# NickTravers/NeuralNetworkLibrary

Measured on AMD Instinct MI355X. Metric: ResNet-34 224x224 training throughput (Learner.train1minibatch, fwd+loss+bwd+optimizer), higher is better.
Workload: dtype f32; 1 GPU; DogsCats ResNet-34 classifier, 224x224, bs=64 per GPU, SGD momentum 0.9, fp32; global_batch=64, image_size=224, parallelism=dp1

## Files before the change

### include/nnl.h

```cpp
#ifndef NNL_H_
#define NNL_H_

#include <stddef.h>
#include <stdint.h>

#ifdef __cplusplus
extern "C" {
#endif

typedef enum {
  NNL_OK = 0,
  NNL_ERR_INVALID_ARG = -1,
  NNL_ERR_HIP = -2,
  NNL_ERR_UNSUPPORTED = -3,
  NNL_ERR_WORKSPACE = -4
} nnl_status_t;

int nnl_version(void);
const char* nnl_last_error(void);
int nnl_reload_env(void);

enum { NNL_PROF_CONV_FWD = 0, NNL_PROF_CONV_DGRAD = 1, NNL_PROF_CONV_WGRAD = 2, NNL_PROF_EMBDOT = 3,
       NNL_PROF_TABULAR = 4, NNL_PROF_RETINA_LOSS = 5, NNL_PROF_LSTM = 6, NNL_PROF_SOFTMAX_CE = 7,
       NNL_PROF_ELEMENTWISE = 8, NNL_PROF_GEMM = 9, NNL_PROF_OPTIM = 10, NNL_PROF_KINDS = 11 };
// ... 62 lines not shown
                            int H, int W, int C, int K, int relu, int flip, void* stream);
int nnl_debug_conv_plan_times(int N, int H, int W, int C, int K, double* out);

int nnl_debug_route_record(int enable);
int nnl_debug_route_collect(char* out, size_t n);
size_t nnl_conv2d_wgrad_workspace_bytes(const nnl_conv_geom_t* g);
int nnl_conv2d_wgrad(const float* x, const float* dy, float* dw, const nnl_conv_geom_t* g, void* workspace,
                     size_t workspace_bytes, void* stream);
size_t nnl_colsum_workspace_bytes(int64_t rows, int64_t cols);
int nnl_sum_tensors(const float* const* src, int n, float* out, int64_t numel, void* stream);
int nnl_colsum(const float* a, float* out, int64_t rows, int64_t cols, void* workspace, size_t workspace_bytes,
               void* stream);
int nnl_relu_gate_colsum(const float* dy, const float* y, float* g, float* colsum, int64_t rows, int64_t cols, void* workspace,
                         size_t workspace_bytes, void* stream);
int nnl_act_gate_colsum(const float* dy, const float* y, float* g, float* colsum, int64_t rows, int64_t cols, int act,
                        void* workspace, size_t workspace_bytes, void* stream);

size_t nnl_bn_workspace_bytes(int64_t rows, int64_t C);
int nnl_bn_fwd(const float* x, const float* gamma, const float* beta, const float* residual, float* y,
               float* save_mean, float* save_invstd, float* running_mean, float* running_var, int64_t rows,
               int64_t C, float eps, float momentum, int training, int relu, int64_t* num_batches_tracked,
               uint32_t* relu_mask, const float* ext_partials, int64_t ext_rows, const float* ext_pivot, float* pivot_out,
               void* workspace, size_t workspace_bytes, void* stream);
int nnl_bn_bwd(const float* dy, const float* y, const uint32_t* relu_mask, const float* x, const float* gamma,
               const float* mean, const float* invstd, float* dx, float* dres, float* dgamma, float* dbeta, int64_t rows,
               int64_t C, int training, int relu, void* workspace, size_t workspace_bytes, void* stream);

int nnl_bn_relu_maxpool_supported(int64_t C);
int nnl_bn_relu_maxpool_fwd(const float* x, const float* gamma, const float* beta, float* y, uint8_t* idx, float* save_mean,
                            float* save_invstd, float* save_scale, float* save_shift, float* running_mean, float* running_var,
                            int64_t N, int64_t H, int64_t W, int64_t C, int64_t P, int64_t Q, int ks, int stride, int pad, float eps,
                            float momentum, int training, int64_t* num_batches_tracked, void* workspace, size_t workspace_bytes,
                            void* stream);
int nnl_bn_relu_maxpool_bwd(const float* dpool, const float* y, const uint8_t* idx, const float* x, const float* gamma,
                            const float* beta, const float* mean, const float* invstd, const float* scale, const float* shift,
                            float* dx, float* dgamma, float* dbeta,
                            int64_t N, int64_t H, int64_t W, int64_t C, int64_t P, int64_t Q, int ks, int stride, int pad,
                            int training, void* workspace, size_t workspace_bytes, void* stream);

int nnl_debug_bn_plan(int64_t rows, int64_t C, int64_t N, int64_t H, int64_t W, int64_t P, int64_t Q, int32_t* out10);

int nnl_bn_sync_stats(const float* x, float* stats, int64_t rows, int64_t C, void* workspace, size_t workspace_bytes,
                      void* stream);
int nnl_bn_sync_fwd(const float* x, const float* all_stats, int world, const float* gamma, const float* beta,
                    const float* residual, float* y, float* save_mean, float* save_invstd, float* running_mean,
                    float* running_var, int64_t rows, int64_t C, float eps, float momentum, int relu,
                    int64_t* num_batches_tracked, uint32_t* relu_mask, void* workspace, size_t workspace_bytes, void* stream);
int nnl_bn_sync_bwd_reduce(const float* dy, const float* y, const uint32_t* relu_mask, const float* x, const float* mean,
                           const float* invstd, float* sums, int64_t rows, int64_t C, int relu, void* workspace,
                           size_t workspace_bytes, void* stream);
int nnl_bn_sync_bwd(const float* dy, const float* y, const uint32_t* relu_mask, const float* x, const float* gamma,
                    const float* mean, const float* invstd, const float* local_sums, const float* global_sums,
                    const float* all_stats,
                    int world, float* dx, float* dres, float* dgamma, float* dbeta, int64_t rows, int64_t C, int relu,
                    void* workspace, size_t workspace_bytes, void* stream);

int nnl_maxpool2d_fwd(const float* x, float* y, uint8_t* idx, int64_t N, int64_t H, int64_t W, int64_t C, int64_t P,
                      int64_t Q, int ksize, int stride, int pad, void* stream);
int nnl_maxpool2d_bwd(const float* dy, const uint8_t* idx, float* dx, int64_t N, int64_t H, int64_t W, int64_t C,
                      int64_t P, int64_t Q, int ksize, int stride, int pad, void* stream);
int nnl_concat_pool_fwd(const float* x, float* out, int32_t* argmax, int64_t N, int64_t HW, int64_t C, void* stream);
int nnl_concat_pool_bwd(const float* dout, const int32_t* argmax, float* dx, int64_t N, int64_t HW, int64_t C, void* stream);

int nnl_bbox_decode(const float* anchors, const float* reg, const float* clas, int64_t bs, int64_t A, int64_t K,
                    const float* mean4, const float* std4, float thresh, float width, float height, float* cand_boxes,
                    int32_t* cand_classes, float* cand_scores, int32_t* cand_order, int32_t* cand_count, void* stream);
// ... 165 lines not shown
```

### neuralnetworklibrary_amd/_lib.py

```python
import ctypes as C
import os

import torch

_HERE = os.path.dirname(os.path.abspath(__file__))
LIB_PATH = os.environ.get('NNL_LIB_PATH') or os.path.join(_HERE, 'libnnl_hip.so')

if not os.path.exists(LIB_PATH):
    raise ImportError(
        f"{LIB_PATH} not found: build it with `python -c 'import __graft_entry__ as g; g.build()'` "
        "(or `make -C neuralnetworklibrary_amd/csrc`). There is no CPU fallback for the HIP hot path.")

lib = C.CDLL(LIB_PATH)

c_p = C.c_void_p
i32, i64, f32, f64 = C.c_int32, C.c_int64, C.c_float, C.c_double
sz = C.c_size_t


class ConvGeom(C.Structure):
    _fields_ = [('N', i32), ('H', i32), ('W', i32), ('C', i32), ('K', i32), ('R', i32), ('S', i32),
                ('stride', i32), ('pad', i32), ('P', i32), ('Q', i32)]


# ... 15 lines not shown
                                     f32, f32, c_p, sz, c_p]),
    'nnl_conv2d_fwd_workspace_bytes': (sz, [C.POINTER(ConvGeom)]),
    'nnl_conv2d_dgrad_workspace_bytes': (sz, [C.POINTER(ConvGeom)]),
    'nnl_conv2d_tile_counters': (i64, []),
    'nnl_conv2d_wino_preferred': (C.c_int, [C.POINTER(ConvGeom), C.c_int]),
    'nnl_wino_filter_multi': (C.c_int, [c_p, c_p, i64, c_p]),
    'nnl_conv2d_fwd_pre': (C.c_int, [c_p, c_p, c_p, c_p, C.POINTER(ConvGeom), C.c_int, c_p, sz, c_p, c_p, c_p, C.POINTER(i32), c_p, c_p]),
    'nnl_conv2d_dgrad_pre': (C.c_int, [c_p, c_p, c_p, C.POINTER(ConvGeom), c_p, c_p, sz, c_p, c_p, c_p]),
    'nnl_debug_conv_wino_workspace_bytes': (sz, [C.c_int] * 5),
    'nnl_debug_conv_wino_fwd': (C.c_int, [c_p] * 6 + [sz, c_p, C.c_long, c_p, c_p] + [C.c_int] * 7 + [c_p]),
    'nnl_debug_conv_wino2_workspace_bytes': (sz, [C.c_int] * 5),
    'nnl_debug_conv_wino2_fwd': (C.c_int, [c_p] * 6 + [sz, c_p, C.c_long, c_p, c_p] + [C.c_int] * 7 + [c_p]),
    'nnl_debug_conv_plan_times': (C.c_int, [C.c_int] * 5 + [C.POINTER(C.c_double)]),
    'nnl_debug_route_record': (C.c_int, [C.c_int]),
    'nnl_debug_route_collect': (C.c_int, [C.c_char_p, sz]),
    'nnl_conv2d_fwd': (C.c_int, [c_p, c_p, c_p, c_p, C.POINTER(ConvGeom), C.c_int, c_p, sz, c_p, c_p, c_p, C.POINTER(i32), c_p]),
    'nnl_conv2d_weight_transpose': (C.c_int, [c_p, c_p, C.c_int, C.c_int, C.c_int, C.c_int, c_p]),
    'nnl_conv2d_weight_transpose_multi': (C.c_int, [c_p, c_p, i64, f64, c_p]),
    'nnl_conv2d_dgrad': (C.c_int, [c_p, c_p, c_p, C.POINTER(ConvGeom), c_p, c_p, sz, c_p, c_p]),
    'nnl_conv2d_wgrad_workspace_bytes': (sz, [C.POINTER(ConvGeom)]),
    'nnl_conv2d_wgrad': (C.c_int, [c_p, c_p, c_p, C.POINTER(ConvGeom), c_p, sz, c_p]),
    'nnl_colsum_workspace_bytes': (sz, [i64, i64]),
    'nnl_colsum': (C.c_int, [c_p, c_p, i64, i64, c_p, sz, c_p]),
    'nnl_relu_gate_colsum': (C.c_int, [c_p, c_p, c_p, c_p, i64, i64, c_p, sz, c_p]),
    'nnl_conv2d_fwd_add_up2': (C.c_int, [c_p, c_p, c_p, c_p, c_p, C.POINTER(ConvGeom), c_p]),
    'nnl_upsample2_bwd': (C.c_int, [c_p, c_p, i64, i64, i64, i64, c_p]),
    'nnl_act_gate_colsum': (C.c_int, [c_p, c_p, c_p, c_p, i64, i64, C.c_int, c_p, sz, c_p]),
    'nnl_maxpool2d_fwd': (C.c_int, [c_p, c_p, c_p, i64, i64, i64, i64, i64, i64, C.c_int, C.c_int, C.c_int, c_p]),
    'nnl_maxpool2d_bwd': (C.c_int, [c_p, c_p, c_p, i64, i64, i64, i64, i64, i64, C.c_int, C.c_int, C.c_int, c_p]),
    'nnl_sum_tensors': (C.c_int, [c_p, C.c_int, c_p, i64, c_p]),
    'nnl_bn_relu_maxpool_supported': (C.c_int, [i64]),
    'nnl_bn_relu_maxpool_fwd': (C.c_int, [c_p, c_p, c_p, c_p, c_p, c_p, c_p, c_p, c_p, c_p, c_p, i64, i64, i64, i64, i64, i64,
                                          C.c_int, C.c_int, C.c_int, f32, f32, C.c_int, c_p, c_p, sz, c_p]),
    'nnl_bn_relu_maxpool_bwd': (C.c_int, [c_p, c_p, c_p, c_p, c_p, c_p, c_p, c_p, c_p, c_p, c_p, c_p, c_p, i64, i64, i64, i64, i64, i64,
                                          C.c_int, C.c_int, C.c_int, C.c_int, c_p, sz, c_p]),
    'nnl_concat_pool_fwd': (C.c_int, [c_p, c_p, c_p, i64, i64, i64, c_p]),
    'nnl_concat_pool_bwd': (C.c_int, [c_p, c_p, c_p, i64, i64, i64, c_p]),
    'nnl_bbox_decode': (C.c_int, [c_p, c_p, c_p, i64, i64, i64, c_p, c_p, f32, f32, f32, c_p, c_p, c_p, c_p, c_p, c_p]),
    'nnl_bbox_decode_window': (C.c_int, [c_p, c_p, c_p, i64, i64, i64, c_p, c_p, f32, f32, f32, f32, f32, c_p, c_p, c_p, c_p, c_p, c_p]),
    'nnl_nms_workspace_bytes': (sz, [i64, i64]),
    'nnl_nms': (C.c_int, [c_p, c_p, c_p, c_p, c_p, i64, i64, i64, f32, c_p, c_p, c_p, c_p, c_p, sz, c_p]),
    'nnl_tta_bbox_merge': (C.c_int, [c_p, c_p, c_p, c_p, c_p, i64, i64, i64, c_p, c_p, c_p, c_p, c_p, c_p, c_p]),
    'nnl_tab_renorm': (C.c_int, [c_p, c_p, c_p, c_p, c_p, c_p, c_p, i64, i32, i32, f32, c_p, c_p]),
    'nnl_tab_gather_fwd': (C.c_int, [c_p, c_p, c_p, c_p, c_p, c_p, c_p, c_p, c_p, c_p, i64, i32, i32, i32, i32, c_p]),
    'nnl_tab_scatter_bwd_workspace_bytes': (sz, [i64, i32]),
    'nnl_tab_scatter_bwd': (C.c_int, [c_p, c_p, c_p, c_p, c_p, c_p, c_p, c_p, c_p, c_p, i64, c_p, i64, i32, i32, i32, i32, c_p, sz, c_p]),
    'nnl_tab_scan_bwd': (C.c_int, [c_p] * 12 + [i32, i32, i64, i32, i32, i32, i32, c_p]),
    'nnl_pad_cols': (C.c_int, [c_p, c_p, i64, i64, i64, c_p]),
    'nnl_keep_masks': (C.c_int, [c_p, c_p, i64, f32, c_p, i64, f32, c_p]),
    'nnl_linear_small_supported': (C.c_int, [i64]),
    'nnl_linear_small_fwd': (C.c_int, [c_p, c_p, c_p, c_p, i64, i64, i64, i64, c_p]),
    'nnl_linear_small_bwd_workspace_bytes': (sz, [i64, i64, i64]),
    'nnl_linear_small_bwd': (C.c_int, [c_p, c_p, c_p, c_p, c_p, c_p, i64, i64, i64, i64, c_p, sz, c_p]),
    'nnl_retina_loss_workspace_bytes': (sz, [i64, i64]),
    'nnl_retina_loss_fwd': (C.c_int, [c_p, c_p, c_p, c_p, c_p, c_p, c_p, c_p, i64, i64, i64, i64, f32, f32, f32, c_p, sz, c_p]),
    'nnl_retina_loss_bwd': (C.c_int, [c_p, c_p, c_p, c_p, c_p, c_p, c_p, c_p, c_p, c_p, i64, i64, i64, i64, f32, f32, f32, c_p]),
    'nnl_lstm_padded_hidden': (i64, [i64]),
    'nnl_lstm_padded_gates': (i64, [i64]),
    'nnl_lstm_workspace_bytes': (sz, [i64, i64, i64]),
    'nnl_lstm_fwd': (C.c_int, [c_p, c_p, c_p, c_p, c_p, c_p, c_p, i64, i64, i64, c_p, sz, c_p, c_p]),
    'nnl_lstm_bwd': (C.c_int, [c_p, c_p, c_p, c_p, c_p, c_p, c_p, c_p, c_p, c_p, i64, i64, i64, c_p, sz, c_p, c_p]),
    'nnl_debug_lstm_bptt2_plan': (C.c_int, [i64, i64, c_p]),
    'nnl_debug_lstm_plan': (C.c_int, [i64, i64, C.POINTER(i32)]),
    'nnl_embedding_rowmask_fwd': (C.c_int, [c_p, c_p, c_p, c_p, i64, i64, i64, c_p, c_p]),
    'nnl_embedding_rowmask_bwd_workspace_bytes': (sz, [i64]),
    'nnl_embedding_rowmask_bwd': (C.c_int, [c_p, c_p, c_p, c_p, i64, i64, i64, i64, c_p, sz, c_p]),
# ... 103 lines not shown
```

### neuralnetworklibrary_amd/csrc/batchnorm.hip

```cpp
#include "nnl_common.h"

namespace {

typedef float f32x4 __attribute__((ext_vector_type(4)));

template <int VEC> struct VecT;
template <> struct VecT<4> { typedef f32x4 type; };
template <> struct VecT<1> { typedef float type; };

template <int VEC> __device__ __forceinline__ float vget(const typename VecT<VEC>::type& v, int i);
template <> __device__ __forceinline__ float vget<4>(const f32x4& v, int i) { return v[i]; }
template <> __device__ __forceinline__ float vget<1>(const float& v, int i) { return v; }
template <int VEC> __device__ __forceinline__ void vset(typename VecT<VEC>::type& v, int i, float x);
template <> __device__ __forceinline__ void vset<4>(f32x4& v, int i, float x) { v[i] = x; }
template <> __device__ __forceinline__ void vset<1>(float& v, int i, float x) { v = x; }

constexpr int kBlock = 256;
constexpr int kMaxRowBlocks = 1024;
constexpr float kCentreAbove = 16.f;
constexpr int kFinLanes = 64;

struct Shape {
  int L;
  int rpb;
// ... 776 lines not shown
    long r = i / g.C4;
    const int w = (int)(r % g.W); r /= g.W;
    const int h = (int)(r % g.H);
    const int n = (int)(r / g.H);
    const f32x4 xv = reinterpret_cast<const f32x4*>(x)[i];
    const f32x4 gg = bnpool_grad(dpool, idx, xv, sc, sh, n, h, w, c4, g);
    f32x4 out;
#pragma unroll
    for (int e = 0; e < 4; ++e) out[e] = ca[e] * gg[e] + cb[e] * xv[e] + cc[e];
    reinterpret_cast<f32x4*>(dx)[i] = out;
  }
}

bool bnpool_ok(long C) { return C % 4 == 0 && C >= 4 && C <= 1024 && (kBlock % (C / 4)) == 0; }
unsigned bnpool_grid(long total) {
  long g = nnl_cdiv(total, (long)kPoolRedBlock * 4);
  if (g > kMaxRowBlocks) g = kMaxRowBlocks;
  return (unsigned)(g < 1 ? 1 : g);
}

int check_stem_geometry(const char* who, long N, long H, long W, long C, long P, long Q, int ks, int stride, int pad) {
  NNL_CHECK_ARG(N > 0 && H > 0 && W > 0 && P > 0 && Q > 0 && ks > 0 && ks * ks <= 255 && stride > 0 && pad >= 0 && 2 * pad <= ks,
                "%s: bad geometry", who);
  NNL_CHECK_ARG(P == (H + 2 * pad - ks) / stride + 1 && Q == (W + 2 * pad - ks) / stride + 1, "%s: P/Q do not match", who);
  NNL_CHECK_ARG(bnpool_ok(C), "%s: C=%ld needs C %% 4 == 0 and C/4 dividing 256", who, C);
  NNL_CHECK_ARG(N * H * W * C < (1L << 31) * 4, "%s: tensor too large", who);
  return NNL_OK;
}

}

extern "C" int nnl_bn_relu_maxpool_supported(int64_t C) { return bnpool_ok(C) ? 1 : 0; }

extern "C" int nnl_bn_relu_maxpool_fwd(const float* x, const float* gamma, const float* beta, float* y, uint8_t* idx,
                                       float* save_mean, float* save_invstd, float* save_scale, float* save_shift,
                                       float* running_mean, float* running_var, int64_t N, int64_t H, int64_t W, int64_t C,
                                       int64_t P, int64_t Q, int ks, int stride, int pad, float eps, float momentum, int training,
                                       int64_t* num_batches_tracked, void* workspace, size_t workspace_bytes, void* stream) {
  NNL_TRY(check_stem_geometry("bn_relu_maxpool_fwd", N, H, W, C, P, Q, ks, stride, pad));
  NNL_CHECK_ARG(x && y && idx && save_mean && save_invstd && save_scale && save_shift, "bn_relu_maxpool_fwd: null pointer");
  NNL_CHECK_ARG(training || (running_mean && running_var), "bn_relu_maxpool_fwd: eval mode needs running statistics");
  const long rows = (long)N * H * W, CG = C / 4;
  Workspace ws;
  NNL_TRY(bind_workspace(workspace, workspace_bytes, rows, C, "bn_relu_maxpool_fwd", ws));
  hipStream_t s = (hipStream_t)stream;
  NnlProfScope prof(NNL_PROF_ELEMENTWISE, s, (double)rows * C * (training ? 8.0 : 4.0) + (double)N * P * Q * C * 5.0);
  const ChannelStats cs{gamma, beta, save_mean, save_invstd, running_mean, running_var, save_scale, save_shift,  nullptr,
                         nullptr, num_batches_tracked, eps, momentum};
  NNL_TRY(launch_channel_affine(x, ws.part, cs, rows, C, training, s));
  const long total = (long)N * P * Q * CG;
  hipLaunchKernelGGL(bnpool_fwd_kernel, dim3((unsigned)nnl_cdiv(total, kBlock)), dim3(kBlock), 0, s, x, save_scale, save_shift, y, idx,
                     (int)N, (int)H, (int)W, (int)CG, (int)P, (int)Q, ks, stride, pad);
  NNL_CHECK_LAUNCH();
  return NNL_OK;
}

extern "C" int nnl_bn_relu_maxpool_bwd(const float* dpool, const float* y, const uint8_t* idx, const float* x, const float* gamma,
                                       const float* beta, const float* mean, const float* invstd, const float* scale,
                                       const float* shift, float* dx, float* dgamma, float* dbeta, int64_t N,
                                       int64_t H, int64_t W, int64_t C, int64_t P, int64_t Q, int ks, int stride, int pad,
                                       int training, void* workspace, size_t workspace_bytes, void* stream) {
  NNL_TRY(check_stem_geometry("bn_relu_maxpool_bwd", N, H, W, C, P, Q, ks, stride, pad));
  NNL_CHECK_ARG(dpool && idx && x && mean && invstd && scale && shift && dx, "bn_relu_maxpool_bwd: null pointer");
  const long rows = (long)N * H * W;
  Workspace ws;
  NNL_TRY(bind_workspace(workspace, workspace_bytes, rows, C, "bn_relu_maxpool_bwd", ws));
  hipStream_t s = (hipStream_t)stream;
  const PoolGeom g{(int)H, (int)W, (int)(C / 4), (int)P, (int)Q, ks, stride, pad};
  const long total = rows * (C / 4);
  NnlProfScope prof(NNL_PROF_ELEMENTWISE, s, (double)rows * C * 12.0 + (double)N * P * Q * C * 10.0);
  unsigned grid;
  if (y != nullptr) {
    grid = bnpool_grid((long)N * P * Q * (C / 4));
    hipLaunchKernelGGL(bnpool_bwd_reduce_out_kernel, dim3(grid), dim3(kPoolRedBlock), 0, s, dpool, y, idx, x, gamma, beta, mean, invstd,
                       ws.part, (int)N, (int)C, g);
  } else {
    grid = bnpool_grid(total);
    hipLaunchKernelGGL(bnpool_bwd_reduce_kernel, dim3(grid), dim3(kPoolRedBlock), 0, s, dpool, idx, x, scale, shift, mean, invstd, ws.part,
                       (int)N, (int)C, g);
  }
  NNL_CHECK_LAUNCH();
  NNL_TRY(launch_bwd_finalize(ws.part, (int)grid, gamma, mean, invstd, dgamma, dbeta, ws.coef, rows, C, training, s));
  hipLaunchKernelGGL(bnpool_bwd_apply_kernel, dim3((unsigned)nnl_cdiv(total, kBlock)), dim3(kBlock), 0, s, dpool, idx, x, scale, shift,
                     ws.coef, dx, (int)N, (int)C, g);
  NNL_CHECK_LAUNCH();
  return NNL_OK;
}
// ... 82 lines not shown
```

### neuralnetworklibrary_amd/csrc/conv2d.hip

```cpp
#include "igemm_kernels.h"
#include "igemm_taps.h"
#include "wino.h"
#include "igemm_wgrad.h"
#include "igemm_wgrad2d.h"

#ifdef NNL_TAPS_TIMING
static void* g_wgrad_dbg = nullptr;
extern "C" void* nnl_debug_wgrad_stamps(void) { return g_wgrad_dbg; }
#endif

namespace {

int check_geom(const nnl_conv_geom_t* g, const char* who) {
  if (!g) return nnl_set_error(NNL_ERR_INVALID_ARG, "%s: null geometry", who);
  if (g->N <= 0 || g->H <= 0 || g->W <= 0 || g->C <= 0 || g->K <= 0 || g->R <= 0 || g->S <= 0 || g->stride <= 0 ||
      g->pad < 0)
    return nnl_set_error(NNL_ERR_INVALID_ARG, "%s: non-positive dimension", who);
  if (g->H + 2L * g->pad < g->R || g->W + 2L * g->pad < g->S)
    return nnl_set_error(NNL_ERR_INVALID_ARG, "%s: the %d x %d filter is larger than the padded input (%d x %d, pad %d)", who, g->R, g->S,
                         g->H, g->W, g->pad);
  const int P = (g->H + 2 * g->pad - g->R) / g->stride + 1, Q = (g->W + 2 * g->pad - g->S) / g->stride + 1;
  if (P != g->P || Q != g->Q || P <= 0 || Q <= 0)
    return nnl_set_error(NNL_ERR_INVALID_ARG, "%s: P,Q=(%d,%d) do not match the geometry (%d,%d)", who, g->P, g->Q, P, Q);
  if (g->C % 4 != 0)
    return nnl_set_error(NNL_ERR_UNSUPPORTED, "%s: C=%d must be a multiple of 4 (pad the channels; ops.py does)", who, g->C);
  if ((long)g->N * g->H * g->W * g->C >= (1L << 31) || (long)g->N * g->P * g->Q * g->K >= (1L << 31) ||
      (long)g->N * g->P * g->Q >= (1L << 30))
    return nnl_set_error(NNL_ERR_UNSUPPORTED, "%s: tensor too large for 32-bit row indexing", who);
  return NNL_OK;
}

template <int BM, int BN, int WGM, int WGN, int MODE>
int launch_rowk(IgemmRowkParams p, hipStream_t s) {
  p.grid_m = (int)nnl_cdiv(p.M, BM);
  p.grid_n = (int)nnl_cdiv(p.Nc, BN);
  NNL_ROUTE("rowk<%d,%d>:%s", BM, BN, MODE == IGEMM_MODE_FWD ? "fwd" : "dgrad");
  hipLaunchKernelGGL((igemm_rowk_kernel<BM, BN, 16, WGM, WGN, MODE>), dim3(p.grid_m * p.grid_n), dim3(256), 0, s, p);
  NNL_CHECK_LAUNCH();
  return NNL_OK;
}

template <int MODE>
int dispatch_rowk(const IgemmRowkParams& p, hipStream_t s) {
  const long b128 = nnl_cdiv(p.M, 128);
  if (p.Nc > 64) {
    if (b128 * nnl_cdiv(p.Nc, 128) >= 400) return launch_rowk<128, 128, 2, 2, MODE>(p, s);
    if (nnl_cdiv(p.M, 64) * nnl_cdiv(p.Nc, 128) >= 400) return launch_rowk<64, 128, 2, 2, MODE>(p, s);
    return launch_rowk<64, 64, 2, 2, MODE>(p, s);
  }
  if (b128 >= 400) return launch_rowk<128, 64, 2, 2, MODE>(p, s);
  return launch_rowk<64, 64, 2, 2, MODE>(p, s);
}


static bool taps_dma(int bk) {
  const int m = NNL_ENV_INT("NNL_IGEMM_DMA", 0);
  return bk == 16 ? (m & 1) != 0 : (m & 2) != 0;
}

template <int BM, int BN, int BK = 16>
int launch_taps(IgemmTapsParams p, hipStream_t s) {
  p.grid_m = (int)nnl_cdiv(p.M, BM);
  p.grid_n = (int)nnl_cdiv(p.Nc, BN);
  p.cls_tiles = p.grid_m * p.grid_n;
  const dim3 grid((unsigned)(p.grid_m * p.grid_n * (p.ncls > 1 ? p.ncls : 1)), p.ksplit > 1 ? p.ksplit : 1);
  NNL_ROUTE("taps<%d,%d,%d>%s%s%s", BM, BN, BK, (BM == 64 && BN == 64 && taps_dma(BK)) ? ":dma" : "", p.ncls > 1 ? ":ncls" : "",
            p.ksplit > 1 ? ":ksplit" : "");
  if constexpr (BM == 64 && BN == 64) {
// ... 803 lines not shown
                                  const float* bn_pivot, int32_t* bn_rows, const float* u, void* stream) {
  if (bn_rows) *bn_rows = 0;
  int st = check_geom(g, "conv2d_fwd");
  if (st) return st;
  NNL_CHECK_ARG(x && w && y, "conv2d_fwd: null pointer");
  NNL_CHECK_ARG(relu >= 0 && relu <= 2, "conv2d_fwd: relu (activation) must be 0 none, 1 ReLU or 2 sigmoid");
  hipStream_t s = (hipStream_t)stream;
  IgemmRowkParams p{};
  p.a = x; p.b = w; p.y = y; p.bias = bias;
  p.N = g->N; p.H = g->H; p.W = g->W; p.C = g->C; p.P = g->P; p.Q = g->Q;
  p.R = g->R; p.S = g->S; p.stride = g->stride; p.pad = g->pad;
  p.M = g->N * g->P * g->Q; p.Nc = g->K; p.Kg = g->R * g->S * g->C; p.relu = relu;
  NnlProfScope prof(NNL_PROF_CONV_FWD, s, 2.0 * p.M * (double)p.Nc * p.Kg);
  const long a_elems = (long)g->N * g->H * g->W * g->C, b_elems = (long)g->K * g->R * g->S * g->C;
  const int wmode = (relu != 2 && workspace != nullptr) ? wino_mode(g->N, g->H, g->W, g->C, g->K, g->R, g->S, g->stride, g->pad) : 0;
  if (wmode && workspace_bytes >= wino_mode_workspace(wmode, g->N, g->H, g->W, g->C, g->K)) {
    WinoProblem wq{};
    wq.in = x; wq.filt = w; wq.out = y; wq.bias = bias; wq.add = nullptr;
    wq.N = g->N; wq.H = g->H; wq.W = g->W; wq.Cin = g->C; wq.Nc = g->K; wq.relu = relu; wq.flip = 0;
    const bool stats = bn_partials && bn_pivot && bn_rows;
    wq.bn_part = stats ? bn_partials : nullptr; wq.bn_pivot = bn_pivot;
    wq.u_pre = u;
    st = wino_mode_launch(wmode, wq, workspace, workspace_bytes, tile_counters, kTileCounters, s);
    if (st == NNL_OK && stats) *bn_rows = wmode >= 2 ? nnl_wino2_bn_rows(g->N, g->H, g->W) : nnl_wino_bn_rows(g->N, g->H, g->W);
    return st;
  }
  if (const int tk = taps_kind(a_elems, b_elems, g->C, g->R * g->S)) {
    IgemmTapsParams q = fwd_taps_params(g, x, w, y, bias, relu);
    q.ktail = tk == 2;
    q.bn_part = (bn_partials && bn_pivot && bn_rows) ? bn_partials : nullptr; q.bn_pivot = bn_pivot;
    return dispatch_taps(q, s, workspace, workspace_bytes, tile_counters, bn_rows);
  }
  if (relu == 2) return nnl_set_error(NNL_ERR_UNSUPPORTED, "conv2d_fwd: the sigmoid epilogue needs C %% 16 == 0 (C=%d)", g->C);
  return dispatch_rowk<IGEMM_MODE_FWD>(p, s);
}

extern "C" int nnl_conv2d_fwd_add_up2(const float* x, const float* w, const float* bias, const float* small, float* y,
                                      const nnl_conv_geom_t* g, void* stream) {
  int st = check_geom(g, "conv2d_fwd_add_up2");
  if (st) return st;
  NNL_CHECK_ARG(x && w && y && small, "conv2d_fwd_add_up2: null pointer");
  NNL_CHECK_ARG(g->P % 2 == 0 && g->Q % 2 == 0, "conv2d_fwd_add_up2: the output (%d x %d) must be twice the small map", g->P, g->Q);
  const long a_elems = (long)g->N * g->H * g->W * g->C, b_elems = (long)g->K * g->R * g->S * g->C;
  if (!taps_ok(a_elems, b_elems, g->C, g->R * g->S))
    return nnl_set_error(NNL_ERR_UNSUPPORTED, "conv2d_fwd_add_up2: needs C %% 16 == 0 (C=%d)", g->C);
  hipStream_t s = (hipStream_t)stream;
  const long M = (long)g->N * g->P * g->Q;
  NnlProfScope prof(NNL_PROF_CONV_FWD, s, 2.0 * M * (double)g->K * g->R * g->S * g->C);
  IgemmTapsParams q = fwd_taps_params(g, x, w, y, bias, 0);
  q.add = small; q.add_up2 = 1;
  return dispatch_taps(q, s);
}

extern "C" int nnl_conv2d_weight_transpose(const float* w, float* wt, int K, int R, int S, int C, void* stream) {
  NNL_CHECK_ARG(w && wt && K > 0 && R > 0 && S > 0 && C > 0, "conv2d_weight_transpose: bad argument");
  hipStream_t s = (hipStream_t)stream;
  NnlProfScope prof(NNL_PROF_ELEMENTWISE, s, 8.0 * K * R * S * C);
  hipLaunchKernelGGL(weight_transpose_kernel, dim3((unsigned)nnl_cdiv(C, 32), (unsigned)nnl_cdiv(K, 32), R * S), dim3(256), 0, s, w,
                     wt, K, R * S, C);
  NNL_CHECK_LAUNCH();
  return NNL_OK;
}

extern "C" int nnl_conv2d_weight_transpose_multi(const nnl_wt_desc_t* desc, const int32_t* tile_tensor, int64_t n_tiles,
                                                 double total_elems, void* stream) {
  NNL_CHECK_ARG(desc && tile_tensor && n_tiles > 0 && n_tiles < (1L << 31), "conv2d_weight_transpose_multi: bad argument");
// ... 261 lines not shown
```

### neuralnetworklibrary_amd/csrc/igemm.h

```cpp
#pragma once
#include "nnl_common.h"

typedef float f32x16 __attribute__((ext_vector_type(16)));
typedef float f32x4 __attribute__((ext_vector_type(4)));

struct IgemmRowkParams {
  const float* a;
  const float* b;
  float* y;
  const float* bias;
  const float* add;
  int N, H, W, C;
  int P, Q;
  int R, S, stride, pad;
  int M, Nc, Kg;
  int relu;
  int grid_m, grid_n;
};

struct IgemmKmajorParams {
  const float* a;
  const float* b;
  float* y;
  int N, H, W, C;
  int P, Q;
  int R, S, stride, pad;
  int Mc, Nc;
  long Kp;
  int splits, k_per_split;
  int grid_m, grid_n;
};

int nnl_internal_gemm_nt(const float* a, const float* b, float* y, const float* bias, const float* add, int M, int N,
                         int K, int relu, hipStream_t s);
int nnl_internal_gemm_nt_splitk(const float* a, const float* b, float* y_slabs, int M, int N, int K, int splits, hipStream_t s);
size_t nnl_internal_gemm_tn_workspace_bytes(int Mc, int Nc, long Kp);
int nnl_internal_gemm_tn(const float* a, const float* b, float* y, int Mc, int Nc, long Kp, void* ws, size_t ws_bytes,
                         hipStream_t s);

__device__ __forceinline__ int nnl_xcd_remap(int bid, int nblk) {
  const int q = nblk >> 3, r = nblk & 7;
  const int xcd = bid & 7, idx = bid >> 3;
  const int base = (xcd < r) ? xcd * (q + 1) : r * (q + 1) + (xcd - r) * q;
  return base + idx;
}
```

### neuralnetworklibrary_amd/csrc/igemm_kernels.h

```cpp
#pragma once
#include "igemm.h"

enum { IGEMM_MODE_FWD = 0, IGEMM_MODE_DGRAD = 1 };

template <int BM, int BN, int BK, int WGM, int WGN, int MODE>
__global__ __launch_bounds__(256) void igemm_rowk_kernel(const IgemmRowkParams p) {
  static_assert(WGM * WGN == 4, "4 waves per block");
  static_assert(BK % 8 == 0, "BK multiple of 8");
  constexpr int BKP = BK + 4;
  constexpr int KC = BK / 4;
  constexpr int RPP = 256 / KC;
  constexpr int PA = BM / RPP, PB = BN / RPP;
  static_assert(PA >= 1 && PB >= 1 && BM % RPP == 0 && BN % RPP == 0, "tile/thread mapping");
  constexpr int WTM = BM / WGM, WTN = BN / WGN;
  constexpr int TM = WTM / 32, TN = WTN / 32;
  static_assert(TM >= 1 && TN >= 1, "wave tile");

  __shared__ __attribute__((aligned(16))) float lds[2][(BM + BN) * BKP];

  const int tid = threadIdx.x, lane = tid & 63, wave = tid >> 6;
  const int wm = wave / WGN, wn = wave % WGN;
  const int logical = nnl_xcd_remap(blockIdx.x, gridDim.x);
  const int tile_m = logical / p.grid_n, tile_n = logical - tile_m * p.grid_n;
  const int m0 = tile_m * BM, n0 = tile_n * BN;

  const int kc = tid % KC, lrow = tid / KC;

  long a_img[PA];
  int a_h0[PA], a_w0[PA];
  const int PQ = p.P * p.Q;
#pragma unroll
  for (int i = 0; i < PA; ++i) {
    const int m = m0 + lrow + i * RPP;
    const bool valid = m < p.M;
    const int mm = valid ? m : 0;
    const int n = mm / PQ;
    const int rem = mm - n * PQ;
    const int pp = rem / p.Q;
    const int qq = rem - pp * p.Q;
    a_img[i] = (long)n * p.H * p.W * p.C;
    if (MODE == IGEMM_MODE_FWD) {
      a_h0[i] = pp * p.stride - p.pad;
      a_w0[i] = qq * p.stride - p.pad;
    } else {
      a_h0[i] = pp + p.pad;
      a_w0[i] = qq + p.pad;
    }
    if (!valid) a_h0[i] = -(1 << 28);
  }
  const float* b_row[PB];
  bool b_ok[PB];
#pragma unroll
  for (int i = 0; i < PB; ++i) {
    const int nr = n0 + lrow + i * RPP;
    b_ok[i] = nr < p.Nc;
    b_row[i] = p.b + (long)(b_ok[i] ? nr : 0) * p.Kg;
  }

  f32x4 ra[PA], rb[PB];
  const f32x4 zero4 = {0.f, 0.f, 0.f, 0.f};

  auto load_tile = [&](int kt) {
    const int k4 = kt * BK + kc * 4;
    const bool kvalid = k4 < p.Kg;
    const int tap = k4 / p.C;
    const int c = k4 - tap * p.C;
    const int r = tap / p.S;
    const int s = tap - r * p.S;
#pragma unroll
    for (int i = 0; i < PA; ++i) {
      int h, w;
      bool ok = kvalid;
      if (MODE == IGEMM_MODE_FWD) {
        h = a_h0[i] + r;
        w = a_w0[i] + s;
      } else {
        const int hh = a_h0[i] - r, ww = a_w0[i] - s;
        if (p.stride == 1) {
          h = hh; w = ww;
        } else {
          ok = ok && hh >= 0 && ww >= 0 && (hh % p.stride == 0) && (ww % p.stride == 0);
          h = hh / p.stride; w = ww / p.stride;
        }
      }
      ok = ok && (unsigned)h < (unsigned)p.H && (unsigned)w < (unsigned)p.W;
      ra[i] = ok ? *reinterpret_cast<const f32x4*>(p.a + a_img[i] + ((long)h * p.W + w) * p.C + c) : zero4;
    }
#pragma unroll
    for (int i = 0; i < PB; ++i)
      rb[i] = (b_ok[i] && kvalid) ? *reinterpret_cast<const f32x4*>(b_row[i] + k4) : zero4;
  };

  auto store_tile = [&](int buf) {
    float* As = lds[buf];
    float* Bs = As + BM * BKP;
// ... 16 lines not shown
    const float* As = lds[buf] + wm * WTM * BKP + frag_off;
    const float* Bs = lds[buf] + BM * BKP + wn * WTN * BKP + frag_off;
#pragma unroll
    for (int kk = 0; kk < BK / 8; ++kk) {
      f32x4 af[TM], bf[TN];
#pragma unroll
      for (int i = 0; i < TM; ++i) af[i] = *reinterpret_cast<const f32x4*>(As + i * 32 * BKP + kk * 8);
#pragma unroll
      for (int j = 0; j < TN; ++j) bf[j] = *reinterpret_cast<const f32x4*>(Bs + j * 32 * BKP + kk * 8);
#pragma unroll
      for (int t = 0; t < 4; ++t)
#pragma unroll
        for (int i = 0; i < TM; ++i)
#pragma unroll
          for (int j = 0; j < TN; ++j)
            acc[i][j] = __builtin_amdgcn_mfma_f32_32x32x2f32(af[i][t], bf[j][t], acc[i][j], 0, 0, 0);
    }
  };

  const int nk = (p.Kg + BK - 1) / BK;
  load_tile(0);
  store_tile(0);
  __syncthreads();
  int cur = 0;
  for (int kt = 0; kt < nk; ++kt) {
    const bool more = kt + 1 < nk;
    if (more) load_tile(kt + 1);
    compute(cur);
    if (more) store_tile(cur ^ 1);
    __syncthreads();
    cur ^= 1;
  }

  const int col_l = lane & 31, row_h = (lane >> 5) * 4;
#pragma unroll
  for (int j = 0; j < TN; ++j) {
    const int col = n0 + wn * WTN + j * 32 + col_l;
    const bool cok = col < p.Nc;
    const float bv = (p.bias != nullptr && cok) ? p.bias[col] : 0.f;
#pragma unroll
    for (int i = 0; i < TM; ++i) {
#pragma unroll
      for (int e = 0; e < 16; ++e) {
        const int row = m0 + wm * WTM + i * 32 + (e & 3) + 8 * (e >> 2) + row_h;
        if (cok && row < p.M) {
          float v = acc[i][j][e] + bv;
          if (p.add) v += p.add[(long)row * p.Nc + col];
          if (p.relu) v = fmaxf(v, 0.f);
          p.y[(long)row * p.Nc + col] = v;
        }
      }
    }
  }
}

template <int BM, int BN, int BK, int WGM, int WGN>
__global__ __launch_bounds__(256) void igemm_kmajor_kernel(const IgemmKmajorParams p) {
  static_assert(WGM * WGN == 4, "4 waves per block");
  constexpr int CA = BM / 4, CB = BN / 4;
  constexpr int RA = 256 / CA, RB = 256 / CB;
  constexpr int PA = BK / RA, PB = BK / RB;
  static_assert(PA >= 1 && PB >= 1 && BK % RA == 0 && BK % RB == 0, "tile/thread mapping");
  constexpr int WTM = BM / WGM, WTN = BN / WGN;
  constexpr int TM = WTM / 32, TN = WTN / 32;
  static_assert(TM >= 1 && TN >= 1, "wave tile");

  __shared__ __attribute__((aligned(16))) float lds[2][BK * (BM + BN)];

  const int tid = threadIdx.x, lane = tid & 63, wave = tid >> 6;
  const int wm = wave / WGN, wn = wave % WGN;
  const int tiles = p.grid_m * p.grid_n;
  const int split = blockIdx.x / tiles;
  const int t_id = blockIdx.x - split * tiles;
  const int tile_n = t_id / p.grid_m, tile_m = t_id - tile_n * p.grid_m;
  const int m0 = tile_m * BM, n0 = tile_n * BN;

  const long k_begin = (long)split * p.k_per_split;
  long k_end = k_begin + p.k_per_split;
  if (k_end > p.Kp) k_end = p.Kp;

  const int ca = tid % CA, ra_row = tid / CA;
  const int a_col = m0 + ca * 4;
  const bool a_cok = a_col < p.Mc;
  const int cb = tid % CB, rb_row = tid / CB;
  const int b_col = n0 + cb * 4;
  const bool b_cok = b_col < p.Nc;
// ... 97 lines not shown
```

### neuralnetworklibrary_amd/ops.py

```python
import collections
import contextlib
import ctypes
import os
import weakref

import numpy as np
import torch

from . import _lib
from ._lib import check, lib, ptr, require_cuda, stream

__all__ = ['mse_loss', 'bce_with_logits', 'fbeta', 'scaled_sigmoid', 'embdotbias', 'index_error_flag', 'raise_if_index_error', 'conv2d', 'to_nhwc', 'from_nhwc', 'linear', 'bn_act', 'concat_pool2d', 'TabularPlan', 'tab_embed_concat', 'embedding_renorm_drop', 'retina_loss', 'image_aug']

_ERR_FLAGS = {}


def _flags(device):
    key = (device.type, device.index)
    if key not in _ERR_FLAGS:
        _ERR_FLAGS[key] = torch.zeros(2, dtype=torch.int32, device=device)
    return _ERR_FLAGS[key]


def index_error_flag(device):
# ... 934 lines not shown


def concat_pool2d(x):
    return _ConcatPool.apply(x)


class _MaxPool2d(torch.autograd.Function):
    @staticmethod
    def forward(ctx, x, ksize, stride, pad):
        require_cuda(x)
        xn = to_nhwc(x.float())
        N, H, W, C = xn.shape
        P, Q = (H + 2 * pad - ksize) // stride + 1, (W + 2 * pad - ksize) // stride + 1
        y = torch.empty(N, P, Q, C, dtype=torch.float32, device=x.device)
        idx = torch.empty(N, P, Q, C, dtype=torch.uint8, device=x.device)
        check(lib.nnl_maxpool2d_fwd(ptr(xn), ptr(y), ptr(idx), N, H, W, C, P, Q, ksize, stride, pad, stream()))
        ctx.save_for_backward(idx)
        ctx.cfg = (N, H, W, C, P, Q, ksize, stride, pad)
        return from_nhwc(y)

    @staticmethod
    def backward(ctx, dy):
        (idx,) = ctx.saved_tensors
        N, H, W, C, P, Q, ksize, stride, pad = ctx.cfg
        dyn = to_nhwc(dy.float())
        dx = torch.empty(N, H, W, C, dtype=torch.float32, device=dy.device)
        check(lib.nnl_maxpool2d_bwd(ptr(dyn), ptr(idx), ptr(dx), N, H, W, C, P, Q, ksize, stride, pad, stream()))
        return from_nhwc(dx), None, None, None


class _BNReLUMaxPool(torch.autograd.Function):

    @staticmethod
    def forward(ctx, x, gamma, beta, running_mean, running_var, training, momentum, eps, nbt, ksize, stride, pad):
        require_cuda(x, gamma, beta)
        xn = to_nhwc(x.float())
        N, H, W, C = xn.shape
        P, Q = (H + 2 * pad - ksize) // stride + 1, (W + 2 * pad - ksize) // stride + 1
        dev = x.device
        y = torch.empty(N, P, Q, C, dtype=torch.float32, device=dev)
        idx = torch.empty(N, P, Q, C, dtype=torch.uint8, device=dev)
        stats = torch.empty(4, C, dtype=torch.float32, device=dev)
        wsb = int(lib.nnl_bn_workspace_bytes(N * H * W, C))
        ws = _workspace(wsb, dev)
        check(lib.nnl_bn_relu_maxpool_fwd(ptr(xn), ptr(gamma), ptr(beta), ptr(y), ptr(idx), ptr(stats[0]), ptr(stats[1]),
                                          ptr(stats[2]), ptr(stats[3]), ptr(running_mean), ptr(running_var), N, H, W, C, P, Q,
                                          ksize, stride, pad, float(eps), float(momentum), int(training), ptr(nbt), ptr(ws), wsb,
                                          stream()))
        ctx.save_for_backward(xn, idx, gamma, beta, stats, y)
        ctx.cfg = (N, H, W, C, P, Q, ksize, stride, pad, training)
        return from_nhwc(y)

    @staticmethod
    def backward(ctx, dy):
        xn, idx, gamma, beta, stats, y = ctx.saved_tensors
        N, H, W, C, P, Q, ksize, stride, pad, training = ctx.cfg
        dyn = to_nhwc(dy.float())
        dx = torch.empty_like(xn)
        dgamma = torch.empty(C, dtype=torch.float32, device=xn.device) if gamma is not None else None
        dbeta = torch.empty(C, dtype=torch.float32, device=xn.device) if gamma is not None else None
        wsb = int(lib.nnl_bn_workspace_bytes(N * H * W, C))
        ws = _workspace(wsb, xn.device)
        check(lib.nnl_bn_relu_maxpool_bwd(ptr(dyn), ptr(y), ptr(idx), ptr(xn), ptr(gamma), ptr(beta), ptr(stats[0]), ptr(stats[1]),
                                          ptr(stats[2]), ptr(stats[3]), ptr(dx), ptr(dgamma), ptr(dbeta), N, H, W, C, P, Q, ksize, stride, pad,
                                          int(training), ptr(ws), wsb, stream()))
        return (from_nhwc(dx), dgamma, dbeta) + (None,) * 9


def conv_bn_relu_maxpool(conv, bn, pool, x):
    k, s, p = pool.kernel_size, pool.stride, pool.padding
    fuse = (x.is_cuda and isinstance(pool, torch.nn.MaxPool2d) and all(isinstance(v, int) for v in (k, s, p))
            and pool.dilation == 1 and not pool.ceil_mode and not pool.return_indices and 2 * p <= k and k * k <= 255
            and not (bn.training and getattr(bn, 'nnl_sync', None) is not None)
            and (bn.running_mean is not None or bn.training)
            and not (bn.training and bn.track_running_stats and bn.momentum is None)
            and bool(lib.nnl_bn_relu_maxpool_supported(bn.num_features)))
    if not fuse:
        return pool(conv_bn_act(conv, bn, x, relu=True))
    y = conv(x)
    training, momentum, nbt, rmean, rvar = _bn_mode(bn)
    return _BNReLUMaxPool.apply(y, bn.weight, bn.bias, rmean, rvar, training, momentum, bn.eps, nbt, k, s, p)


def maxpool2d(x, ksize=3, stride=2, pad=1):
    return _MaxPool2d.apply(x, int(ksize), int(stride), int(pad))


class TabularPlan:

    def __init__(self, weights):
        dev = weights[0].device
        self.key = tuple((w.data_ptr(), tuple(w.shape)) for w in weights) + (str(dev),)
        self.sync = None
        card = [int(w.shape[0]) for w in weights]
        dim = [int(w.shape[1]) for w in weights]
        self.ncat, self.cat_width, self.total_rows = len(weights), sum(dim), sum(card)
        col_off = np.concatenate([[0], np.cumsum(dim)[:-1]]).astype(np.int32)
        row_off = np.concatenate([[0], np.cumsum(card)[:-1]]).astype(np.int32)
        sizes = [c * d for c, d in zip(card, dim)]
        self.grad_sizes, self.shapes = sizes, [tuple(w.shape) for w in weights]
        grad_off = np.concatenate([[0], np.cumsum(sizes)[:-1]]).astype(np.int64)
        self.grad_elems = int(sum(sizes))
        t = lambda a, dt: torch.as_tensor(np.asarray(a), dtype=dt).to(dev)
        self.ptrs = t(np.array([w.data_ptr() for w in weights], dtype=np.int64), torch.int64)
        self.card, self.dim = t(card, torch.int32), t(dim, torch.int32)
        self.col_off, self.row_off, self.grad_off = t(col_off, torch.int32), t(row_off, torch.int32), t(grad_off, torch.int64)
        self.col_table = t(np.repeat(np.arange(self.ncat), dim), torch.int32)
        self.row_table = t(np.repeat(np.arange(self.ncat), card), torch.int32)
        self.flags = torch.zeros(self.total_rows, dtype=torch.int32, device=dev)
        self.max_dim = max(dim) if dim else 0
        blk_col, blk_first = [], []
        for j, n in enumerate(sizes):
            for f in range(0, n, 256):
                blk_col.append(j)
# ... 242 lines not shown
```

Baseline: 5547 images/s.

## Fuse BN statistics into stem conv epilogue and use buffer loads for stem

Adds a stem-specialised rowk igemm kernel for the 7x7 stride-2 C=4 conv. It writes per-64-row partial sums of (v - pivot) and (v - pivot)^2 from the epilogue, and it uses raw buffer loads with out-of-range offsets in place of per-element bounds branches. The fused BN+ReLU+maxpool forward can then finalize statistics from these partials instead of rereading the full conv output. Pivots are cached on the BN module from the previous step, which adds a workspace write and an LDS reduction to the conv epilogue.

Result: no change. 5561 images/s, median of 6 (+0.2%).

```diff
diff --git a/include/nnl.h b/include/nnl.h
--- a/include/nnl.h
+++ b/include/nnl.h
@@ -118,6 +118,11 @@
                             int64_t N, int64_t H, int64_t W, int64_t C, int64_t P, int64_t Q, int ks, int stride, int pad, float eps,
                             float momentum, int training, int64_t* num_batches_tracked, void* workspace, size_t workspace_bytes,
                             void* stream);
+int nnl_bn_relu_maxpool_fwd_ext(const float* x, const float* gamma, const float* beta, float* y, uint8_t* idx, float* save_mean,
+                                float* save_invstd, float* save_scale, float* save_shift, float* running_mean, float* running_var,
+                                int64_t N, int64_t H, int64_t W, int64_t C, int64_t P, int64_t Q, int ks, int stride, int pad, float eps,
+                                float momentum, int training, int64_t* num_batches_tracked, const float* ext_partials, int64_t ext_rows,
+                                const float* ext_pivot, float* pivot_out, void* workspace, size_t workspace_bytes, void* stream);
 int nnl_bn_relu_maxpool_bwd(const float* dpool, const float* y, const uint8_t* idx, const float* x, const float* gamma,
                             const float* beta, const float* mean, const float* invstd, const float* scale, const float* shift,
                             float* dx, float* dgamma, float* dbeta,
diff --git a/neuralnetworklibrary_amd/_lib.py b/neuralnetworklibrary_amd/_lib.py
--- a/neuralnetworklibrary_amd/_lib.py
+++ b/neuralnetworklibrary_amd/_lib.py
@@ -71,6 +71,8 @@
     'nnl_bn_relu_maxpool_supported': (C.c_int, [i64]),
     'nnl_bn_relu_maxpool_fwd': (C.c_int, [c_p, c_p, c_p, c_p, c_p, c_p, c_p, c_p, c_p, c_p, c_p, i64, i64, i64, i64, i64, i64,
                                           C.c_int, C.c_int, C.c_int, f32, f32, C.c_int, c_p, c_p, sz, c_p]),
+    'nnl_bn_relu_maxpool_fwd_ext': (C.c_int, [c_p, c_p, c_p, c_p, c_p, c_p, c_p, c_p, c_p, c_p, c_p, i64, i64, i64, i64, i64, i64,
+                                              C.c_int, C.c_int, C.c_int, f32, f32, C.c_int, c_p, c_p, i64, c_p, c_p, c_p, sz, c_p]),
     'nnl_bn_relu_maxpool_bwd': (C.c_int, [c_p, c_p, c_p, c_p, c_p, c_p, c_p, c_p, c_p, c_p, c_p, c_p, c_p, i64, i64, i64, i64, i64, i64,
                                           C.c_int, C.c_int, C.c_int, C.c_int, c_p, sz, c_p]),
     'nnl_concat_pool_fwd': (C.c_int, [c_p, c_p, c_p, i64, i64, i64, c_p]),
diff --git a/neuralnetworklibrary_amd/csrc/batchnorm.hip b/neuralnetworklibrary_amd/csrc/batchnorm.hip
--- a/neuralnetworklibrary_amd/csrc/batchnorm.hip
+++ b/neuralnetworklibrary_amd/csrc/batchnorm.hip
@@ -832,11 +832,13 @@
 
 extern "C" int nnl_bn_relu_maxpool_supported(int64_t C) { return bnpool_ok(C) ? 1 : 0; }
 
-extern "C" int nnl_bn_relu_maxpool_fwd(const float* x, const float* gamma, const float* beta, float* y, uint8_t* idx,
-                                       float* save_mean, float* save_invstd, float* save_scale, float* save_shift,
-                                       float* running_mean, float* running_var, int64_t N, int64_t H, int64_t W, int64_t C,
-                                       int64_t P, int64_t Q, int ks, int stride, int pad, float eps, float momentum, int training,
-                                       int64_t* num_batches_tracked, void* workspace, size_t workspace_bytes, void* stream) {
+extern "C" int nnl_bn_relu_maxpool_fwd_ext(const float* x, const float* gamma, const float* beta, float* y, uint8_t* idx,
+                                           float* save_mean, float* save_invstd, float* save_scale, float* save_shift,
+                                           float* running_mean, float* running_var, int64_t N, int64_t H, int64_t W, int64_t C,
+                                           int64_t P, int64_t Q, int ks, int stride, int pad, float eps, float momentum, int training,
+                                           int64_t* num_batches_tracked, const float* ext_partials, int64_t ext_rows,
+                                           const float* ext_pivot, float* pivot_out, void* workspace, size_t workspace_bytes,
+                                           void* stream) {
   NNL_TRY(check_stem_geometry("bn_relu_maxpool_fwd", N, H, W, C, P, Q, ks, stride, pad));
   NNL_CHECK_ARG(x && y && idx && save_mean && save_invstd && save_scale && save_shift, "bn_relu_maxpool_fwd: null pointer");
   NNL_CHECK_ARG(training || (running_mean && running_var), "bn_relu_maxpool_fwd: eval mode needs running statistics");
@@ -846,13 +848,26 @@
   hipStream_t s = (hipStream_t)stream;
   NnlProfScope prof(NNL_PROF_ELEMENTWISE, s, (double)rows * C * (training ? 8.0 : 4.0) + (double)N * P * Q * C * 5.0);
   const ChannelStats cs{gamma, beta, save_mean, save_invstd, running_mean, running_var, save_scale, save_shift,  nullptr,
-                         nullptr, num_batches_tracked, eps, momentum};
-  NNL_TRY(launch_channel_affine(x, ws.part, cs, rows, C, training, s));
+                        training ? pivot_out : nullptr, num_batches_tracked, eps, momentum};
+  if (training && ext_partials != nullptr && ext_rows > 0 && ext_pivot != nullptr)
+    NNL_TRY(launch_finalize(ext_pivot, ext_partials, (int)ext_rows, true, cs, rows, C, s));
+  else
+    NNL_TRY(launch_channel_affine(x, ws.part, cs, rows, C, training, s));
   const long total = (long)N * P * Q * CG;
   hipLaunchKernelGGL(bnpool_fwd_kernel, dim3((unsigned)nnl_cdiv(total, kBlock)), dim3(kBlock), 0, s, x, save_scale, save_shift, y, idx,
                      (int)N, (int)H, (int)W, (int)CG, (int)P, (int)Q, ks, stride, pad);
   NNL_CHECK_LAUNCH();
   return NNL_OK;
+}
+
+extern "C" int nnl_bn_relu_maxpool_fwd(const float* x, const float* gamma, const float* beta, float* y, uint8_t* idx,
+                                       float* save_mean, float* save_invstd, float* save_scale, float* save_shift,
+                                       float* running_mean, float* running_var, int64_t N, int64_t H, int64_t W, int64_t C,
+                                       int64_t P, int64_t Q, int ks, int stride, int pad, float eps, float momentum, int training,
+                                       int64_t* num_batches_tracked, void* workspace, size_t workspace_bytes, void* stream) {
+  return nnl_bn_relu_maxpool_fwd_ext(x, gamma, beta, y, idx, save_mean, save_invstd, save_scale, save_shift, running_mean, running_var, N, H,
+                                     W, C, P, Q, ks, stride, pad, eps, momentum, training, num_batches_tracked, nullptr, 0, nullptr, nullptr,
+                                     workspace, workspace_bytes, stream);
 }
 
 extern "C" int nnl_bn_relu_maxpool_bwd(const float* dpool, const float* y, const uint8_t* idx, const float* x, const float* gamma,
diff --git a/neuralnetworklibrary_amd/csrc/conv2d.hip b/neuralnetworklibrary_amd/csrc/conv2d.hip
--- a/neuralnetworklibrary_amd/csrc/conv2d.hip
+++ b/neuralnetworklibrary_amd/csrc/conv2d.hip
@@ -30,10 +30,23 @@
   return NNL_OK;
 }
 
+bool stem_geometry(const nnl_conv_geom_t* g) {
+  return g->R == 7 && g->S == 7 && g->stride == 2 && g->pad == 3 && g->C == 4 && g->K % 64 == 0 &&
+         (long)g->N * g->H * g->W * 16 < (1L << 31) && (long)g->K * 196 * 4 < (1L << 31);
+}
+
 template <int BM, int BN, int WGM, int WGN, int MODE>
 int launch_rowk(IgemmRowkParams p, hipStream_t s) {
   p.grid_m = (int)nnl_cdiv(p.M, BM);
   p.grid_n = (int)nnl_cdiv(p.Nc, BN);
+  if constexpr (MODE == IGEMM_MODE_FWD) {
+    if (p.bn_part != nullptr) {
+      NNL_ROUTE("rowk<%d,%d>:fwd:bn_stats", BM, BN);
+      hipLaunchKernelGGL((igemm_rowk_stem_kernel<BM, BN, 16, WGM, WGN>), dim3(p.grid_m * p.grid_n), dim3(256), 0, s, p);
+      NNL_CHECK_LAUNCH();
+      return NNL_OK;
+    }
+  }
   NNL_ROUTE("rowk<%d,%d>:%s", BM, BN, MODE == IGEMM_MODE_FWD ? "fwd" : "dgrad");
   hipLaunchKernelGGL((igemm_rowk_kernel<BM, BN, 16, WGM, WGN, MODE>), dim3(p.grid_m * p.grid_n), dim3(256), 0, s, p);
   NNL_CHECK_LAUNCH();
@@ -903,6 +916,12 @@
     return dispatch_taps(q, s, workspace, workspace_bytes, tile_counters, bn_rows);
   }
   if (relu == 2) return nnl_set_error(NNL_ERR_UNSUPPORTED, "conv2d_fwd: the sigmoid epilogue needs C %% 16 == 0 (C=%d)", g->C);
+  if (stem_geometry(g) && bias == nullptr && relu == 0 && bn_partials && bn_pivot && bn_rows && NNL_ENV_INT("NNL_CONV_STEM", 1) != 0) {
+    p.bn_part = bn_partials; p.bn_pivot = bn_pivot;
+    st = dispatch_rowk<IGEMM_MODE_FWD>(p, s);
+    if (st == NNL_OK) *bn_rows = (int32_t)nnl_cdiv(p.M, 64);
+    return st;
+  }
   return dispatch_rowk<IGEMM_MODE_FWD>(p, s);
 }
 
diff --git a/neuralnetworklibrary_amd/csrc/igemm.h b/neuralnetworklibrary_amd/csrc/igemm.h
--- a/neuralnetworklibrary_amd/csrc/igemm.h
+++ b/neuralnetworklibrary_amd/csrc/igemm.h
@@ -16,6 +16,8 @@
   int M, Nc, Kg;
   int relu;
   int grid_m, grid_n;
+  float* bn_part;
+  const float* bn_pivot;
 };
 
 struct IgemmKmajorParams {
diff --git a/neuralnetworklibrary_amd/csrc/igemm_kernels.h b/neuralnetworklibrary_amd/csrc/igemm_kernels.h
--- a/neuralnetworklibrary_amd/csrc/igemm_kernels.h
+++ b/neuralnetworklibrary_amd/csrc/igemm_kernels.h
@@ -3,8 +3,13 @@
 
 enum { IGEMM_MODE_FWD = 0, IGEMM_MODE_DGRAD = 1 };
 
-template <int BM, int BN, int BK, int WGM, int WGN, int MODE>
-__global__ __launch_bounds__(256) void igemm_rowk_kernel(const IgemmRowkParams p) {
+typedef int i32x4 __attribute__((ext_vector_type(4)));
+__device__ __forceinline__ f32x4 rowk_buf_load4(__amdgpu_buffer_rsrc_t rsrc, unsigned voff) {
+  return __builtin_bit_cast(f32x4, __builtin_bit_cast(i32x4, __builtin_amdgcn_raw_buffer_load_b128(rsrc, (int)voff, 0, 0)));
+}
+
+template <int BM, int BN, int BK, int WGM, int WGN, int MODE, bool STEM>
+__device__ __forceinline__ void igemm_rowk_body(const IgemmRowkParams& p) {
   static_assert(WGM * WGN == 4, "4 waves per block");
   static_assert(BK % 8 == 0, "BK multiple of 8");
   constexpr int BKP = BK + 4;
@@ -28,6 +33,7 @@
 
   long a_img[PA];
   int a_h0[PA], a_w0[PA];
+  unsigned a_tap0[PA];
   const int PQ = p.P * p.Q;
 #pragma unroll
   for (int i = 0; i < PA; ++i) {
@@ -46,6 +52,7 @@
       a_h0[i] = pp + p.pad;
       a_w0[i] = qq + p.pad;
     }
+    if constexpr (STEM) a_tap0[i] = (unsigned)((n * p.H + a_h0[i]) * p.W + a_w0[i]) * 16u;
     if (!valid) a_h0[i] = -(1 << 28);
   }
   const float* b_row[PB];
@@ -56,11 +63,29 @@
     b_ok[i] = nr < p.Nc;
     b_row[i] = p.b + (long)(b_ok[i] ? nr : 0) * p.Kg;
   }
+  const __amdgpu_buffer_rsrc_t ra_src = __builtin_amdgcn_make_buffer_rsrc(const_cast<float*>(p.a), 0, STEM ? p.N * p.H * p.W * 16 : 0, 0x00020000);
+  const __amdgpu_buffer_rsrc_t rb_src = __builtin_amdgcn_make_buffer_rsrc(const_cast<float*>(p.b), 0, STEM ? p.Nc * 196 * 4 : 0, 0x00020000);
 
   f32x4 ra[PA], rb[PB];
   const f32x4 zero4 = {0.f, 0.f, 0.f, 0.f};
 
   auto load_tile = [&](int kt) {
+    if constexpr (STEM) {
+      static_assert(MODE == IGEMM_MODE_FWD, "the stem specialisation is a forward kernel");
+      const int tap = kt * KC + kc;
+      const bool kvalid = tap < 49;
+      const int r = tap / 7, s = tap - r * 7;
+      const unsigned koff = (unsigned)(r * p.W + s) * 16u;
+#pragma unroll
+      for (int i = 0; i < PA; ++i) {
+        const bool ok = kvalid && (unsigned)(a_h0[i] + r) < (unsigned)p.H && (unsigned)(a_w0[i] + s) < (unsigned)p.W;
+        ra[i] = rowk_buf_load4(ra_src, ok ? a_tap0[i] + koff : 0xFFFFFFFFu);
+      }
+#pragma unroll
+      for (int i = 0; i < PB; ++i)
+        rb[i] = rowk_buf_load4(rb_src, (b_ok[i] && kvalid) ? (unsigned)((n0 + lrow + i * RPP) * 196 + tap * 4) * 4u : 0xFFFFFFFFu);
+      return;
+    }
     const int k4 = kt * BK + kc * 4;
     const bool kvalid = k4 < p.Kg;
     const int tap = k4 / p.C;
@@ -143,14 +168,19 @@
     cur ^= 1;
   }
 
+  static_assert(!STEM || (BM % 64 == 0 && (BM / 64) * BN <= 256 && (BM / 32) * BN * 2 <= 2 * (BM + BN) * BKP), "statistics epilogue mapping");
+  float* red = &lds[0][0];
   const int col_l = lane & 31, row_h = (lane >> 5) * 4;
 #pragma unroll
   for (int j = 0; j < TN; ++j) {
     const int col = n0 + wn * WTN + j * 32 + col_l;
     const bool cok = col < p.Nc;
     const float bv = (p.bias != nullptr && cok) ? p.bias[col] : 0.f;
+    float piv = 0.f;
+    if constexpr (STEM) piv = cok ? p.bn_pivot[col] : 0.f;
 #pragma unroll
     for (int i = 0; i < TM; ++i) {
+      float s1 = 0.f, s2 = 0.f;
 #pragma unroll
       for (int e = 0; e < 16; ++e) {
         const int row = m0 + wm * WTM + i * 32 + (e & 3) + 8 * (e >> 2) + row_h;
@@ -159,10 +189,43 @@
           if (p.add) v += p.add[(long)row * p.Nc + col];
           if (p.relu) v = fmaxf(v, 0.f);
           p.y[(long)row * p.Nc + col] = v;
+          if constexpr (STEM) {
+            const float d = v - piv;
+            s1 += d; s2 += d * d;
+          }
         }
       }
-    }
-  }
+      if constexpr (STEM) {
+        s1 += __shfl_xor(s1, 32, 64);
+        s2 += __shfl_xor(s2, 32, 64);
+        if (lane < 32) {
+          const int o = (((wm * WTM) / 32 + i) * BN + wn * WTN + j * 32 + col_l) * 2;
+          red[o] = s1; red[o + 1] = s2;
+        }
+      }
+    }
+  }
+  if constexpr (STEM) {
+    __syncthreads();
+    const int grp = tid / BN, cl = tid - grp * BN;
+    if (grp < BM / 64 && m0 + grp * 64 < p.M && n0 + cl < p.Nc) {
+      const float* lo = red + ((2 * grp) * BN + cl) * 2;
+      const float* hi = red + ((2 * grp + 1) * BN + cl) * 2;
+      float* out = p.bn_part + ((long)(m0 / 64 + grp) * p.Nc + n0 + cl) * 2;
+      out[0] = lo[0] + hi[0];
+      out[1] = lo[1] + hi[1];
+    }
+  }
+}
+
+template <int BM, int BN, int BK, int WGM, int WGN, int MODE>
+__global__ __launch_bounds__(256) void igemm_rowk_kernel(const IgemmRowkParams p) {
+  igemm_rowk_body<BM, BN, BK, WGM, WGN, MODE, false>(p);
+}
+
+template <int BM, int BN, int BK, int WGM, int WGN>
+__global__ __launch_bounds__(256) void igemm_rowk_stem_kernel(const IgemmRowkParams p) {
+  igemm_rowk_body<BM, BN, BK, WGM, WGN, IGEMM_MODE_FWD, true>(p);
 }
 
 template <int BM, int BN, int BK, int WGM, int WGN>
diff --git a/neuralnetworklibrary_amd/ops.py b/neuralnetworklibrary_amd/ops.py
--- a/neuralnetworklibrary_amd/ops.py
+++ b/neuralnetworklibrary_amd/ops.py
@@ -990,7 +990,8 @@
 class _BNReLUMaxPool(torch.autograd.Function):
 
     @staticmethod
-    def forward(ctx, x, gamma, beta, running_mean, running_var, training, momentum, eps, nbt, ksize, stride, pad):
+    def forward(ctx, x, gamma, beta, running_mean, running_var, training, momentum, eps, nbt, ksize, stride, pad, ext=None,
+                pivot_out=None):
         require_cuda(x, gamma, beta)
         xn = to_nhwc(x.float())
         N, H, W, C = xn.shape
@@ -1001,10 +1002,11 @@
         stats = torch.empty(4, C, dtype=torch.float32, device=dev)
         wsb = int(lib.nnl_bn_workspace_bytes(N * H * W, C))
         ws = _workspace(wsb, dev)
-        check(lib.nnl_bn_relu_maxpool_fwd(ptr(xn), ptr(gamma), ptr(beta), ptr(y), ptr(idx), ptr(stats[0]), ptr(stats[1]),
-                                          ptr(stats[2]), ptr(stats[3]), ptr(running_mean), ptr(running_var), N, H, W, C, P, Q,
-                                          ksize, stride, pad, float(eps), float(momentum), int(training), ptr(nbt), ptr(ws), wsb,
-                                          stream()))
+        check(lib.nnl_bn_relu_maxpool_fwd_ext(ptr(xn), ptr(gamma), ptr(beta), ptr(y), ptr(idx), ptr(stats[0]), ptr(stats[1]),
+                                              ptr(stats[2]), ptr(stats[3]), ptr(running_mean), ptr(running_var), N, H, W, C, P, Q,
+                                              ksize, stride, pad, float(eps), float(momentum), int(training), ptr(nbt),
+                                              ptr(ext[0]) if ext else None, (ext[0].numel() // (2 * C)) if ext else 0,
+                                              ptr(ext[1]) if ext else None, ptr(pivot_out), ptr(ws), wsb, stream()))
         ctx.save_for_backward(xn, idx, gamma, beta, stats, y)
         ctx.cfg = (N, H, W, C, P, Q, ksize, stride, pad, training)
         return from_nhwc(y)
@@ -1022,7 +1024,7 @@
         check(lib.nnl_bn_relu_maxpool_bwd(ptr(dyn), ptr(y), ptr(idx), ptr(xn), ptr(gamma), ptr(beta), ptr(stats[0]), ptr(stats[1]),
                                           ptr(stats[2]), ptr(stats[3]), ptr(dx), ptr(dgamma), ptr(dbeta), N, H, W, C, P, Q, ksize, stride, pad,
                                           int(training), ptr(ws), wsb, stream()))
-        return (from_nhwc(dx), dgamma, dbeta) + (None,) * 9
+        return (from_nhwc(dx), dgamma, dbeta) + (None,) * 11
 
 
 def conv_bn_relu_maxpool(conv, bn, pool, x):
@@ -1035,9 +1037,25 @@
             and bool(lib.nnl_bn_relu_maxpool_supported(bn.num_features)))
     if not fuse:
         return pool(conv_bn_act(conv, bn, x, relu=True))
-    y = conv(x)
     training, momentum, nbt, rmean, rvar = _bn_mode(bn)
-    return _BNReLUMaxPool.apply(y, bn.weight, bn.bias, rmean, rvar, training, momentum, bn.eps, nbt, k, s, p)
+
+    def pooled(y, ext=None, pivot_out=None):
+        return _BNReLUMaxPool.apply(y, bn.weight, bn.bias, rmean, rvar, training, momentum, bn.eps, nbt, k, s, p, ext, pivot_out)
+    stats = (bn.training and bn.track_running_stats and bn.running_mean is not None and getattr(conv, 'nnl_hip_conv', False)
+             and conv.bias is None and not conv.fuse_relu and conv.dilation == (1, 1) and conv.groups == 1
+             and conv.stride[0] == conv.stride[1] and conv.padding[0] == conv.padding[1] and conv.padding_mode == 'zeros'
+             and torch.is_grad_enabled() and os.environ.get('NNL_BN_EPI_STATS', '1') != '0')
+    if not stats:
+        return pooled(conv(x))
+    pivot = getattr(bn, '_nnl_pivot', None)
+    if pivot is None or pivot.device != x.device or pivot.numel() != bn.num_features:
+        if torch.cuda.is_current_stream_capturing():
+            return pooled(conv(x))
+        pivot = torch.empty(bn.num_features, dtype=torch.float32, device=x.device)
+        object.__setattr__(bn, '_nnl_pivot', pivot)
+        return pooled(conv(x), pivot_out=pivot)
+    y, part = conv2d_with_bn_stats(x, conv.weight, None, conv.stride[0], conv.padding[0], pivot)
+    return pooled(y, ext=(part, pivot) if part.numel() > 0 else None, pivot_out=pivot)
 
 
 def maxpool2d(x, ksize=3, stride=2, pad=1):
```
